# y9c/cutseq

Measured on AMD Instinct MI355X. Metric: M read-pairs/sec, higher is better.
Workload: dtype u8

## Files before the change

cutseq_amd/csrc/cutseq_hip.hip:

```cpp
#include <hip/hip_runtime.h>

#include <cstdarg>
#include <cstdio>
#include <cstdlib>
#include <cstring>
#include <algorithm>
#include <atomic>
#include <map>
#include <new>
#include <string>
#include <thread>
#include <vector>

#include <sys/mman.h>

#include "../../include/cutseq_hip.h"
#include "trim_kernel.hip.inc"
#include "long_kernel.hip.inc"
#include "text_kernels.hip.inc"
#include "deflate_kernels.hip.inc"
#include "info_kernels.hip.inc"

namespace {

// ... 82 lines not shown
}

struct cs_engine {
  int device = -1;
  hipStream_t stream = nullptr;
  int plan_slot = -1;
  hipStream_t resolve_stream = nullptr;
  unsigned long long *d_stats = nullptr;
  Lane lanes[kLanes];
  int next_lane = 0;
  Lane *last_lane = nullptr;
  uint32_t timed_calls = 0;
  double kernel_ms_total[2] = {0, 0};
  uint32_t max_reads = 0, max_stride = 0;
  bool paired = false;
  bool coded = false;
  bool wide = false;
  bool max_n = false;
  int n_cus = 256;
  uint32_t n_table_ops = 1;
  uint32_t col_dwords = 0;
  uint32_t waves_per_simd[2] = {4, 4};
  bool long_demux = false;
  int demux_mate = -1;
  uint32_t info_adapters = 0, info_max_m = 0, info_uniq_flags = 0;
  uint32_t demux_bins = 0;
  std::vector<Slot> slots;
  uint32_t max_dynamic_lds[2] = {0, 0};
  std::vector<void *> d_tables;
  uint32_t knob_col_bytes = 0, knob_grid_x = 0, knob_batch = 1;
  uint32_t knob_resolve_waves = 4;
  uint32_t knob_item_slots = 0;
  uint32_t knob_fast_recode = 1;
  bool knob_units = false;
  uint32_t knob_big_shift = 0, knob_small_shift = 0, knob_big_pct = 50;
};

namespace {

bool is_acgt(uint8_t c) { return c == 'A' || c == 'C' || c == 'G' || c == 'T'; }

void sync_fields(csdev::DevOp &d) {
  const cs_op &o = d.op;
  csdev::DevFields &f = d.f;
  f.kind = o.kind, f.align_flags = o.align_flags, f.reversed = o.reversed, f.remove = o.remove, f.shortcut = o.shortcut;
  f.match_flag = o.match_flag, f.required = o.required, f.conditional = o.conditional, f.capture = o.capture;
  f.homopolymer = o.homopolymer, f.q_base = o.q_base, f.stat_slot = o.stat_slot, f.m = o.m, f.k = o.k;
  f.min_overlap = o.min_overlap, f.force_min_len = o.force_min_len, f.cut_len = o.cut_len, f.q_cutoff = o.q_cutoff;
}

int build_dev_op(const cs_op &in, csdev::DevOp &out, int index, int mate) {
  memset(&out, 0, sizeof out);
  out.op = in;
  cs_op &op = out.op;
  switch (op.kind) {
    case CS_OP_ADAPTER: {
      if (op.m < 1 || op.m > CS_MAX_ADAPTER) return fail(CS_ERR_ARG, "mate %d op %d: adapter length %u", mate, index, op.m);
      if (op.min_overlap < 1 || op.min_overlap > op.m)
        return fail(CS_ERR_ARG, "mate %d op %d: min_overlap %u not in [1, m]", mate, index, op.min_overlap);
      if (op.align_flags > 15) return fail(CS_ERR_ARG, "mate %d op %d: bad align_flags", mate, index);
      if (op.k > op.m || op.thr[op.m] != op.k)
        return fail(CS_ERR_ARG, "mate %d op %d: k=%u inconsistent with thr[m]=%u", mate, index, op.k, op.thr[op.m]);
      for (int i = 1; i <= op.m; ++i)
        if (op.thr[i] < op.thr[i - 1] || op.thr[i] > op.thr[i - 1] + 1)
          return fail(CS_ERR_ARG, "mate %d op %d: thr[] must be a non-decreasing unit-step table", mate, index);
      if (op.remove > 1 || op.shortcut > 1) return fail(CS_ERR_ARG, "mate %d op %d: bad remove/shortcut", mate, index);
// ... 151 lines not shown
    a.mate[m].bc = rr[m]->bc;
    a.mate[m].xflags = rr[m]->xflags;
  }
  Lane &ln = eng->lanes[eng->next_lane];
  eng->next_lane = (eng->next_lane + 1) % kLanes;
  if (ln.used && hipEventQuery(ln.done) != hipSuccess) HIP_TRY(hipStreamWaitEvent(stream, ln.done, 0));
  if (n_reads > ln.defer_capacity) {
    const uint32_t cap = n_reads + n_reads / 8 + 1024;
    for (Lane &l : eng->lanes) {
      if (cap <= l.defer_capacity) continue;
      if (l.used) HIP_TRY(hipEventSynchronize(l.done));
      for (int m = 0; m < 2; ++m) {
        if (l.d_defer[m]) (void)hipFree(l.d_defer[m]);
        l.d_defer[m] = nullptr;
      }
      l.defer_capacity = 0;
      for (uint32_t m = 0; m < (eng->paired ? 2u : 1u); ++m)
        HIP_TRY(hipMalloc(&l.d_defer[m], (size_t)cap * kDeferRecordBytes));
      l.defer_capacity = cap;
    }
  }
  a.defer[0] = reinterpret_cast<uint4 *>(ln.d_defer[0]);
  a.defer[1] = reinterpret_cast<uint4 *>(ln.d_defer[1]);
  a.defer_count = ln.d_counters + kTileCounterDwords;
  a.defer_cap = ln.defer_capacity;
  a.stats = eng->d_stats;
  a.n_reads = n_reads;
  a.stride_dw = stride / 4;
  a.plan_slot = (uint32_t)eng->plan_slot;
  a.tile_counter = ln.d_counters;
  a.n_table_ops = eng->n_table_ops;
  a.batch_knob = eng->knob_batch;
  a.fast_recode = eng->knob_fast_recode;
  a.gate = gate;
  for (int mode = 0; mode < 2; ++mode)
    if (g[mode].lds_bytes > eng->max_dynamic_lds[mode]) {
      HIP_TRY(hipFuncSetAttribute(kernel_for(eng, mode), hipFuncAttributeMaxDynamicSharedMemorySize, (int)g[mode].lds_bytes));
      eng->max_dynamic_lds[mode] = g[mode].lds_bytes;
    }
  const uint32_t n_tiles = (n_reads + kTileRows - 1) / kTileRows;
  uint32_t gx[2];
  for (int mode = 0; mode < 2; ++mode) {
    uint32_t per_cu = kLdsBudget / g[mode].lds_bytes;
    const uint32_t wave_cap = 4 * eng->waves_per_simd[mode];
    if (per_cu > wave_cap) per_cu = wave_cap;
    if (per_cu < 1) per_cu = 1;
    if (mode == csdev::MODE_RESOLVE && rstream != stream && per_cu > eng->knob_resolve_waves) per_cu = eng->knob_resolve_waves;
    uint32_t resident = (uint32_t)eng->n_cus * per_cu * (mode == csdev::MODE_SCAN ? 2u : 1u);
    gx[mode] = resident / mates;
    if (mode == csdev::MODE_SCAN && eng->knob_grid_x) gx[mode] = eng->knob_grid_x;
    if (gx[mode] < 1) gx[mode] = 1;
    if (gx[mode] > n_tiles) gx[mode] = n_tiles;
  }
  a.static_units = gx[0] / 2 > 0 ? gx[0] / 2 : 1;
  const uint32_t share = n_tiles / a.static_units;
  a.big_shift = share >= 32 ? 3 : share >= 16 ? 2 : 1;
  a.small_shift = 0;
  uint32_t big_pct = 50;
  if (eng->knob_units) {
    a.big_shift = eng->knob_big_shift;
    a.small_shift = eng->knob_small_shift;
    big_pct = eng->knob_big_pct;
  }
  a.big_tiles = (uint32_t)((uint64_t)n_tiles * big_pct / 100) & ~((1u << a.big_shift) - 1u);
  if (time_it) {
    int rc = harvest(eng, ln);
// ... 572 lines not shown
  const size_t bytes = (size_t)max_reads * max_stride;
  for (Slot &s : eng->slots) {
    for (int m = 0; m < (eng->paired ? 2 : 1); ++m) {
      ENG_TRY(hipMalloc(&s.d_seq[m], bytes));
      ENG_TRY(hipMalloc(&s.d_qual[m], bytes));
      ENG_TRY(hipMalloc(&s.d_len[m], (size_t)max_reads * sizeof(uint16_t)));
      ENG_TRY(hipMalloc(&s.d_out[m], (size_t)max_reads * sizeof(cs_result)));
      ENG_TRY(hipMalloc(&s.d_bc[m], (size_t)max_reads));
      if (eng->max_n) ENG_TRY(hipMalloc(&s.d_xf[m], (size_t)max_reads));
    }
    ENG_TRY(hipMalloc(&s.d_cap2, (size_t)max_reads * sizeof(cs_cap2)));
    ENG_TRY(hipEventCreateWithFlags(&s.done, hipEventDisableTiming));
  }
  ENG_TRY(hipDeviceSynchronize());
#undef ENG_TRY
  for (int mode = 0; mode < 2; ++mode) {
    hipFuncAttributes fa;
    if (hipFuncGetAttributes(&fa, kernel_for(eng, mode)) == hipSuccess && fa.numRegs > 0) {
      const uint32_t alloc = ((uint32_t)fa.numRegs + 7u) / 8u * 8u;
      uint32_t w = 512u / alloc;
      eng->waves_per_simd[mode] = w < 1 ? 1 : (w > 8 ? 8 : w);
    }
  }
  if (const char *env = getenv("CUTSEQ_COL_BYTES")) {
    const long v = atol(env);
    if (v >= 1024 && v <= 32768) eng->knob_col_bytes = (uint32_t)v;
  }
  if (const char *env = getenv("CUTSEQ_BATCH_KNOB")) eng->knob_batch = (uint32_t)atol(env);
  if (const char *env = getenv("CUTSEQ_ITEM_SLOTS")) {
    const long v = atol(env);
    if (v >= 1 && v <= 16) eng->knob_item_slots = (uint32_t)v;
  }
  if (const char *env = getenv("CUTSEQ_FAST_RECODE")) eng->knob_fast_recode = (uint32_t)atoi(env) <= 2u ? (uint32_t)atoi(env) : 1u;
  if (const char *env = getenv("CUTSEQ_RESOLVE_WAVES")) {
    const long v = atol(env);
    if (v >= 1 && v <= 16) eng->knob_resolve_waves = (uint32_t)v;
  }
  if (const char *env = getenv("CUTSEQ_GRID_X")) {
    const long v = atol(env);
    if (v > 0) eng->knob_grid_x = (uint32_t)v;
  }
  if (const char *env = getenv("CUTSEQ_UNITS")) {
    unsigned bs, ss, pc;
    if (sscanf(env, "%u,%u,%u", &bs, &ss, &pc) == 3 && bs <= 6 && ss <= bs && pc <= 100) {
      eng->knob_units = true;
      eng->knob_big_shift = bs;
      eng->knob_small_shift = ss;
      eng->knob_big_pct = pc;
    }
  }
  *out = eng;
  return CS_OK;
}

int cs_trim_device(cs_engine *eng, void *stream, const cs_reads *r1, const cs_reads *r2, uint32_t n_reads,
                   uint32_t stride) {
  if (!eng || !r1) return fail(CS_ERR_ARG, "null engine or reads");
  HIP_TRY(hipSetDevice(eng->device));
  hipStream_t st = stream ? (hipStream_t)stream : eng->stream;
  return launch(eng, st, st, r1, r2, n_reads, stride, true);
}

int cs_trim_device_pipelined(cs_engine *eng, void *stream, const cs_reads *r1, const cs_reads *r2, uint32_t n_reads,
                             uint32_t stride) {
  if (!eng || !r1) return fail(CS_ERR_ARG, "null engine or reads");
  HIP_TRY(hipSetDevice(eng->device));
// ... 850 lines not shown
```

cutseq_amd/csrc/trim_kernel.hip.inc:

```

#include <type_traits>

namespace csdev {

#ifdef CS_PHASE_TIMERS
struct PhaseTimer {
  uint64_t last;
  uint32_t acc[8];
  uint32_t passes, steps, items;
};
#define CS_T_MARK(T, PHASE)                                   \
  {                                                           \
    const uint64_t cs_now = clock64();                        \
    (T).acc[PHASE] += (uint32_t)(cs_now - (T).last);          \
    (T).last = cs_now;                                        \
  }
#else
#define CS_T_MARK(T, PHASE)
#endif


constexpr int kWave = 64;

constexpr uint32_t kScoreBias = 1024u, kOriginBias = 4096u;
// ... 54 lines not shown

struct MateArgs {
  const uint32_t *seq;
  const uint8_t *qual;
  const uint16_t *len;
  cs_result *out;
  cs_cap2 *cap2;
  uint8_t *bc;
  uint8_t *xflags;
};

constexpr uint32_t kTileCounters = 8, kTileCounterStride = 32;

struct KArgs {
  MateArgs mate[2];
  unsigned long long *stats;
  uint32_t n_reads;
  uint32_t stride_dw;
  uint32_t lds_stride_dw;
  uint32_t col_dwords;
  uint32_t plan_slot;
  uint32_t *tile_counter;
  uint32_t n_table_ops;
  uint32_t big_tiles;
  uint32_t big_shift, small_shift;
  uint32_t static_units;
  uint4 *defer[2];
  uint32_t batch_knob;
  uint32_t *defer_count;
  uint32_t defer_cap;
  const unsigned long long *gate;
  uint32_t item_slots;
  uint32_t fast_recode;
};

__device__ __forceinline__ uint32_t cell_pack(int cost, int score, int origin) {
  return ((uint32_t)cost << kCostShift) | ((uint32_t)(score + (int)kScoreBias) << kScoreShift) |
         (uint32_t)(origin + (int)kOriginBias);
}
__device__ __forceinline__ int cell_cost(uint32_t c) { return (int)(c >> kCostShift); }
__device__ __forceinline__ int cell_score(uint32_t c) { return (int)((c >> kScoreShift) & 0x7ffu) - (int)kScoreBias; }
__device__ __forceinline__ int cell_origin(uint32_t c) { return (int)(c & 0x1fffu) - (int)kOriginBias; }
constexpr uint32_t kStripScoreBias = 256u, kStripPrioShift = 22;
constexpr uint32_t kStripZero = (kStripScoreBias << kScoreShift) | kOriginBias;
__device__ __forceinline__ uint32_t strip_pack(int cost, int score, int origin) {
  return ((uint32_t)cost << kCostShift) | ((uint32_t)(score + (int)kStripScoreBias) << kScoreShift) |
         (uint32_t)(origin + (int)kOriginBias);
}
__device__ __forceinline__ int strip_score(uint32_t c) {
  return (int)((c >> kScoreShift) & 0x1ffu) - (int)kStripScoreBias;
}

__device__ __forceinline__ int thr_of(const DevOp &d, int L) {
  if (d.thr_mul) return (int)(__umul24((uint32_t)max(L, 0), d.thr_mul) >> 16);
  if (L <= 0) return 0;
  if (L <= 64) return __popcll(d.thr_step[0] & (~0ull >> (64 - L)));
  return __popcll(d.thr_step[0]) + __popcll(d.thr_step[1] & (~0ull >> (128 - L)));
}
__device__ __forceinline__ int thr_step_bit(const DevOp &d, int i) {
  return (int)(((i <= 64) ? (d.thr_step[0] >> (i - 1)) : (d.thr_step[1] >> (i - 65))) & 1ull);
}

__device__ __forceinline__ uint32_t encode4_nib(uint32_t w) {
  const uint32_t sel = (w >> 1) & 0x03030303u;
  const uint32_t expect = __builtin_amdgcn_perm(0u, 0x47544341u , sel);
  const uint32_t diff = expect ^ w;
  const uint32_t nz = (((diff & 0x7f7f7f7fu) + 0x7f7f7f7fu) | diff) & 0x80808080u;
// ... 164 lines not shown
  const W Xh = (((Eq & Pv) + Pv) ^ Pv) | Eq;
  W Ph = Mv | ~(Xh | Pv);
  W Mh = Pv & Xh;
  st.score += (int)((Ph >> top_shift) & 1) - (int)((Mh >> top_shift) & 1);
  Ph = (Ph << 1) | hin;
  Mh = Mh << 1;
  st.Pv = Mh | ~(Xv | Ph);
  st.Mv = Ph & Xv;
}

__device__ __forceinline__ uint32_t shl1_full_rate(uint32_t x) {
  uint32_t r;
  asm("v_add_u32 %0, %1, %1" : "=v"(r) : "v"(x));
  return r;
}
constexpr uint32_t kTtA = 0xF0u, kTtB = 0xCCu, kTtC = 0xAAu;
template <bool HIN>
__device__ __forceinline__ void myers_step_la(MyersState<uint32_t> &st, uint32_t Eq, uint32_t hin_bit) {
  const uint32_t Pv = st.Pv, Mv = st.Mv;
  const uint32_t Xv = Eq | Mv;
  const uint32_t t = (Eq & Pv) + Pv;
  const uint32_t Xh = __builtin_amdgcn_bitop3_b32(t, Pv, Eq, ((kTtA ^ kTtB) | kTtC) & 0xFFu);
  const uint32_t Ph = __builtin_amdgcn_bitop3_b32(Mv, Xh, Pv, (kTtA | ~(kTtB | kTtC)) & 0xFFu);
  const uint32_t Mh = Pv & Xh;
  st.score += (int)(Ph >> 31) - (int)(Mh >> 31);
  uint32_t Ph2 = shl1_full_rate(Ph);
  if (HIN) Ph2 |= hin_bit;
  const uint32_t Mh2 = shl1_full_rate(Mh);
  st.Pv = __builtin_amdgcn_bitop3_b32(Mh2, Xv, Ph2, (kTtA | ~(kTtB | kTtC)) & 0xFFu);
  st.Mv = Ph2 & Xv;
}

typedef __attribute__((address_space(3))) const uint32_t lds_cu32;
__device__ __forceinline__ uint32_t lds_addr_of(const void *p) {
  return (uint32_t)(uintptr_t)(__attribute__((address_space(3))) const void *)p;
}
__device__ __forceinline__ uint32_t lds_read_u32(uint32_t addr) { return *(lds_cu32 *)(uintptr_t)addr; }

constexpr int kFnibDwords = 6;
#ifndef PRIO_LOOP
#define PRIO_LOOP 0
#define PRIO_REST 3
#define PRIO_RESOLVE 3
#endif
constexpr int kRingRecords = 16;

__device__ __forceinline__ int hamming_coded(const uint32_t *row, int p0, const uint32_t *fnib, int f0, int L, int m) {
  const int rw = p0 >> 3, fw = f0 >> 3;
  const uint32_t rsh = (uint32_t)(p0 & 7) * 4u, fsh = (uint32_t)(f0 & 7) * 4u;
  uint32_t rd[5], fd[5];
#pragma unroll
  for (int q = 0; q < 5; ++q) {
    if (8 * (q - 1) >= m) break;
    rd[q] = row[rw + q];
    fd[q] = fnib[fw + q];
  }
  int diff = 0;
#pragma unroll
  for (int q = 0; q < 4; ++q) {
    if (8 * q >= m) break;
    const uint32_t r = __builtin_amdgcn_alignbit(rd[q + 1], rd[q], rsh);
    const uint32_t f = __builtin_amdgcn_alignbit(fd[q + 1], fd[q], fsh);
    uint32_t x = r ^ f;
    x |= x >> 1;
    x |= x >> 2;
    x &= 0x11111111u;
// ... 560 lines not shown
    bool any = false;
    for (int i = skip + 1; i <= m; ++i) {
      cost += (int)(pv & 1u) - (int)(mv & 1u);
      pv >>= 1;
      mv >>= 1;
      thr_i += thr_step_bit(d, i);
      any = any || cost <= thr_i;
    }
    none = none && !any;
  }
  return none;
}

__device__ __forceinline__ unsigned long long lds_read_u64(uint32_t addr) { return *(const lds_u64 *)(uintptr_t)addr; }
typedef __attribute__((address_space(3))) uint8_t lds_u8;
__device__ __forceinline__ void lds_write_u8(uint32_t addr, uint32_t imm, uint32_t value) {
  *(lds_u8 *)(uintptr_t)(addr + imm) = (uint8_t)value;
}
__device__ __forceinline__ uint32_t lds_read_u8(uint32_t addr) { return *(const lds_u8 *)(uintptr_t)addr; }
__device__ __forceinline__ uint32_t pk_min_u16(uint32_t a, uint32_t b) {
  uint32_t r;
  asm("v_pk_min_u16 %0, %1, %2" : "=v"(r) : "v"(a), "v"(b));
  return r;
}

struct ItemLog {
  uint32_t slot0;
  uint32_t bytes;
  uint32_t tag_off;
};

template <bool HAS_A>
__device__ __forceinline__ Verdict myers_pair(const DevOp &da, const DevOp &db, int rule, const uint32_t *fnib_b,
                                               const uint32_t *row, int e, bool &a_none, const ItemLog &il CS_T_PARAM) {
  constexpr int NB = 8;
  constexpr int s = 0;
  const int n = e - s;
  const int m = db.f.m, k = db.f.k;
  const bool RS = db.f.align_flags & CS_REF_START;
  const int sh = 32 - m;
  MyersState<uint32_t> st;
  st.Mv = 0;
  st.Pv = RS ? 0u : (m >= 32 ? ~0u : ((1u << m) - 1u));
  const int k1 = k + 1;
  st.score = (RS ? 0 : m) - k1;
  st.Pv = (st.Pv << sh) | ((1u << sh) - 1u);
  const bool exact_by_score = !RS;
  int jfirst = -1, jlast = -1;
  int cmin = 0x7fff, jmin = -1;
  bool tie_next = false;
  uint32_t slot = il.slot0;
  const uint32_t slot_end = il.slot0 + il.bytes;
  bool log_full = false;
  const int ma = da.f.m, ka = da.f.k;
  const int sha = 32 - ma, free_a = ma - (int)da.f.min_overlap;
  MyersState<uint32_t> sa;
  sa.Mv = 0;
  sa.Pv = (((ma >= 32 ? ~0u : ((1u << ma) - 1u)) & ~((1u << free_a) - 1u)) << sha) | ((1u << sha) - 1u);
  sa.score = ma - free_a;
  int flag = 0;
  const uint32_t tn0 = da.pair_tn[0], tn1 = da.pair_tn[1], tn2 = da.pair_tn[2], tn3 = da.pair_tn[3];
  const uint32_t fill_a = (uint32_t)sha, cst4 = (uint32_t)(4 + 2 * ka + 1);
  auto sample_a = [&](uint32_t cst) {
    const int cur = (int)__builtin_popcount(sa.Pv) - (int)(__builtin_popcount(sa.Mv) + fill_a);
    flag |= sa.score + cur - (int)cst;
    sa.score = cur;
  };
  const unsigned long long tn_lo = ((unsigned long long)tn1 << 32) | tn0, tn_hi = ((unsigned long long)tn3 << 32) | tn2;
  auto tn_of = [tn_lo, tn_hi, ka](int j) -> int {
    int t1 = ka + 1;
    if (__ballot(j <= 32)) {
      const unsigned long long w = j <= 16 ? tn_lo : tn_hi;
      const int tj = (int)((uint32_t)(w >> (((uint32_t)(j - 1) & 15u) * 4u)) & 15u);
      t1 = j > 32 ? t1 : tj;
    }
    return t1;
  };
  auto column = [&](uint32_t eb, uint32_t ea, int j) {
    myers_step_la<false>(st, eb, 0u);
    if constexpr (HAS_A) {
      myers_step_la<false>(sa, ea, 0u);
      flag |= sa.score - tn_of(j);
    }
    if (st.score < 0) {
      if (jfirst < 0) jfirst = j;
      jlast = j;
      if (j == jmin + 1 && st.score + k1 == cmin) tie_next = true;
      if (st.score + k1 < cmin) {
        cmin = st.score + k1;
        jmin = j;
        tie_next = false;
      }
    }
  };
  int j = 1;
  if (n >= NB) {
    int wi = 0;
    auto take = [&]() -> uint32_t { return row[wi]; };
    auto advance = [&]() { wi += 1; };
#ifndef CS_PAIR_DEPTH
#define CS_PAIR_DEPTH 2
#endif
    constexpr int QD = CS_PAIR_DEPTH;
    static_assert(NB % QD == 0, "a group's columns must map onto the slots the same way in every group");
    uint32_t qb[QD], qa[QD];
    auto refill = [&](int slot, uint32_t code) {
      const unsigned long long pr = lds_read_u64(code);
      qb[slot] = (uint32_t)pr;
      qa[slot] = (uint32_t)(pr >> 32);
    };
    uint32_t wcur = take();
    advance();
#pragma unroll
    for (int u = 0; u < QD; ++u) refill(u, word_code<true>(wcur, u));
    auto group = [&](auto early_tag, uint32_t tw) {
      constexpr bool EARLY = decltype(early_tag)::value;
      const uint32_t wnext = take();
      advance();
      int sc[NB];
#pragma unroll
      for (int u = 0; u < NB; ++u) {
        myers_step_la<false>(st, qb[u % QD], 0u);
        sc[u] = st.score;
        if constexpr (HAS_A && EARLY) {
          myers_step_la<false>(sa, qa[u % QD], 0u);
          flag |= sa.score - (int)((tw >> (4 * u)) & 15u);
        } else if constexpr (HAS_A) {
          myers_step_noscore<false>(sa, qa[u % QD], 0u);
          if (u == 3 || u == 7) sample_a(cst4);
        }
        refill(u % QD, u + QD < NB ? word_code<true>(wcur, u + QD) : word_code<true>(wnext, u + QD - NB));
      }
      wcur = wnext;
      constexpr uint32_t kOr3 = 0xFEu;
      uint32_t any = __builtin_amdgcn_bitop3_b32((uint32_t)sc[0], (uint32_t)sc[1], (uint32_t)sc[2], kOr3);
      any = __builtin_amdgcn_bitop3_b32(any, (uint32_t)sc[3], (uint32_t)sc[4], kOr3);
      any = __builtin_amdgcn_bitop3_b32(any, (uint32_t)sc[5], (uint32_t)sc[6], kOr3);
      any |= (uint32_t)sc[7];
      if ((int)any < 0) {
        if (slot < slot_end) {
#pragma unroll
          for (int u = 0; u < NB; ++u) lds_write_u8(slot, (uint32_t)u, (uint32_t)sc[u]);
          lds_write_u8((slot >> 3) + il.tag_off, 0u, (uint32_t)(j >> 3));
        }
        slot += 8u;
      }
      j += NB;
    };
    __builtin_amdgcn_s_setprio(PRIO_LOOP);
    const int early_groups = (ma + ka + NB - 1) >> 3;
    if constexpr (HAS_A) {
      int g = 0;
      do {
        group(std::true_type{}, g == 0 ? tn0 : g == 1 ? tn1 : g == 2 ? tn2 : tn3);
        ++g;
      } while (g < early_groups && j + NB - 1 <= n);
    }
    while (j + NB - 1 <= n) group(std::false_type{}, 0u);
    __builtin_amdgcn_s_setprio(PRIO_REST);
    if (j <= n) {
      int sc[NB];
#pragma unroll
      for (int u = 0; u < NB - 1; ++u) {
        sc[u] = 0x7f;
        if (j + u <= n) {
          uint32_t eb, ea;
          if (u < QD) {
            eb = qb[u];
            ea = qa[u];
          } else {
            const unsigned long long pr = lds_read_u64(word_code<true>(wcur, u));
            eb = (uint32_t)pr;
            ea = (uint32_t)(pr >> 32);
          }
          myers_step_la<false>(st, eb, 0u);
          sc[u] = st.score;
          if constexpr (HAS_A) {
            myers_step_la<false>(sa, ea, 0u);
            flag |= sa.score - tn_of(j + u);
          }
        }
      }
      sc[NB - 1] = 0x7f;
      int any = sc[0];
#pragma unroll
      for (int u = 1; u < NB - 1; ++u) any |= sc[u];
      if (any < 0) {
        if (slot < slot_end) {
#pragma unroll
          for (int u = 0; u < NB; ++u) lds_write_u8(slot, (uint32_t)u, (uint32_t)sc[u]);
          lds_write_u8((slot >> 3) + il.tag_off, 0u, (uint32_t)(j >> 3));
        }
        slot += 8u;
      }
      j = n + 1;
    }
    {
      const uint32_t m80 = 0x80808080u, ones = 0x01010101u;
      const uint32_t stop_at = min(slot, slot_end);
      uint32_t rd = il.slot0;
      while (__ballot(rd < stop_at)) {
        if (rd < stop_at) {
          const unsigned long long sc8 = lds_read_u64(rd);
          const int jg = (int)lds_read_u8((rd >> 3) + il.tag_off) * 8 + 1;
          rd += 8u;
          const uint32_t clo = (uint32_t)sc8 & m80, chi = (uint32_t)(sc8 >> 32) & m80;
          const uint32_t plo = (uint32_t)sc8 ^ m80, phi = (uint32_t)(sc8 >> 32) ^ m80;
          const unsigned long long c64 = ((unsigned long long)chi << 32) | clo;
          if (jfirst < 0) jfirst = jg + (__builtin_ctzll(c64) >> 3);
          jlast = jg + ((63 - __builtin_clzll(c64)) >> 3);
          const uint32_t h00ff = 0x00ff00ffu;
          const uint32_t a0 = plo & h00ff, a1 = (plo >> 8) & h00ff, b0 = phi & h00ff, b1 = (phi >> 8) & h00ff;
          const uint32_t m4 = pk_min_u16(pk_min_u16(a0, a1), pk_min_u16(b0, b1));
          const uint32_t gbyte = min(m4 & 0xffffu, m4 >> 16);
          const int gmin = (int)gbyte - 128 + k1;
          if (jmin == jg - 1 && (int)(plo & 0xffu) - 128 + k1 == cmin) tie_next = true;
          if (gmin < cmin) {
            const uint32_t gb = __builtin_amdgcn_perm(0u, gbyte, 0u);
            const uint32_t xlo = plo ^ gb, xhi = phi ^ gb;
            const uint32_t zlo = (xlo - ones) & ~xlo & m80, zhi = (xhi - ones) & ~xhi & m80;
            const int pos = __builtin_ctzll(((unsigned long long)zhi << 32) | zlo) >> 3;
            cmin = gmin;
            jmin = jg + pos;
            const unsigned long long flipped = ((unsigned long long)phi << 32) | plo;
            tie_next = pos < 7 && (uint32_t)((flipped >> (8 * (pos + 1))) & 0xffull) == gbyte;
          }
        }
// ... 850 lines not shown
  const uint32_t big_mask = (1u << a.big_shift) - 1u, small_mask = (1u << a.small_shift) - 1u;
  auto unit_start = [&](uint32_t u) -> uint32_t {
    return (u < big_units) ? (u << a.big_shift) : big_tiles + ((u - big_units) << a.small_shift);
  };
  auto unit_end = [&](uint32_t tile) -> uint32_t {
    return (tile < big_tiles) ? ((tile | big_mask) + 1u) : big_tiles + (((tile - big_tiles) | small_mask) + 1u);
  };
  uint32_t *next_slot = sacc + kStatWords;
  const uint32_t n_counters = min(kTileCounters, (uint32_t)gridDim.x);
  const uint32_t my_counter = blockIdx.x % n_counters;
  uint32_t *counter = a.tile_counter + ((uint32_t)mate * kTileCounters + my_counter) * kTileCounterStride;
  uint32_t *claim = a.defer_count + (2u + (uint32_t)mate) * kTileCounterStride;
  auto next_unit = [&]() -> uint32_t { return a.static_units + my_counter + n_counters * atomicAdd(counter, 1u); };
  if (SCAN) {
    if (tid == 0) *next_slot = unit_start(blockIdx.x < a.static_units ? blockIdx.x : next_unit());
  } else {
    if (tid == 0) *next_slot = atomicAdd(claim, 1u);
  }
  __syncthreads();
  uint32_t tile_id = *next_slot, next_id = 0;
#ifdef CS_PHASE_TIMERS
  PhaseTimer pt;
  pt.last = clock64();
  for (int i = 0; i < 8; ++i) pt.acc[i] = 0;
  pt.passes = pt.steps = pt.items = 0;
#endif

  uint4 *ring = reinterpret_cast<uint4 *>((reinterpret_cast<uintptr_t>(sacc + kStatWords + 4) + 15u) & ~(uintptr_t)15u);
  uint32_t pend_count = 0;
  bool pend_asked = false;
  uint32_t pend_q = 0;
  auto flush_ring = [&]() {
    const uint32_t qb = (uint32_t)__builtin_amdgcn_readfirstlane((int)pend_q);
    if ((uint32_t)lane < pend_count) {
      uint4 *rec = a.defer[mate] + (size_t)(qb + (uint32_t)lane) * 2u;
      rec[0] = ring[lane * 2];
      rec[1] = ring[lane * 2 + 1];
    }
    pend_count = 0;
    pend_asked = false;
  };
  bool fast_ok = SCAN && CODED && a.fast_recode != 0u, fast_failed = false;
  for (; tile_id < n_tiles; tile_id = next_id) {
  uint32_t lane_fresh = threadIdx.x;
  asm volatile("" : "+v"(lane_fresh));
  const int tid = (int)lane_fresh, lane = tid;
  const bool top = !SCAN && tile_id >= tiles_a;
  const uint32_t row0 = top ? (tile_id - tiles_a) * (uint32_t)TILE : tile_id * batch_rows;
  const uint32_t rows_here = top ? min((uint32_t)TILE, n_refl - row0) : min(batch_rows, (SCAN ? a.n_reads : n_records) - row0);
  const bool valid = (uint32_t)tid < rows_here;

  uint32_t gr = row0 + tid;
  int s = 0, e = 0, t0 = 0;
  uint32_t fm = 0, capo = 0, qc = 0;
  uint32_t meta = (uint32_t)CS_DEMUX_NONE << 16;
  uint32_t rec_win = 0, rec_rows = 0, rec_rmax = 0;
  if (!SCAN) {
    uint4 ra = make_uint4(0, 0, 0, 0), rb = make_uint4(0, 0, 0, 0);
    if (valid) {
      const uint4 *rec = a.defer[mate] + (size_t)(top ? a.defer_cap - 1u - gr : gr) * 2u;
      ra = rec[0];
      rb = rec[1];
    }
    gr = ra.x;
    s = (int)(ra.y & 0xffffu);
    e = (int)(ra.y >> 16);
    rec_win = ra.z;
    rec_rows = ra.w;
    t0 = (int)(rb.x >> 24);
    fm = (rb.y & 0xffu) | ((rb.x & 0xffffffu) << 8);
    meta = ((rb.y >> 8) & 0xffu) | ((rb.w >> 24) << 16);
    rec_rmax = (rb.y >> 16) & 0xffu;
    capo = rb.z;
    qc = ((rb.w >> 8) & 0xffffu) | ((rb.y >> 24) << 16) | (rb.w << 24);
  }

  const uint32_t len_raw = valid ? (uint32_t)ma.len[gr] : 0u;
// ... 136 lines not shown
  if (tid == 0 && !same_unit) fetched = SCAN ? atomic_add_later(counter, 1u) : atomic_add_later(claim, 1u);
  if (SCAN && pend_count >= (uint32_t)kRingRecords / 2) {
    if (tid == 0) pend_q = atomic_add_later(&a.defer_count[mate * kTileCounterStride], pend_count);
    pend_asked = true;
  }
  const uint32_t *wave_rows = tile;
  const uint32_t *myrow = wave_rows + (size_t)lane * a.lds_stride_dw;
  bool deferred = false;
  bool refl = false;
  bool refl_any = false;
  uint32_t refl_q = 0, refl_rank = 0;

  if (SCAN) e = len;
  int t_first = 0;
  if constexpr (SCAN && CODED) {
    const bool pair = use_filter && n_ops >= 2 && plan->ops[mate][0].pair_next;
    const bool solo = use_filter && n_ops >= 1 && plan->ops[mate][0].solo_first;
    if (pair || solo) {
      const int tb = pair ? 1 : 0;
      const DevOp &da = plan->ops[mate][0], &db = plan->ops[mate][tb];
      if (lane < 8) {
        cur_tab[lane * 2] = tables[tb * (kEqTableBytes / 4) + lane * 2 + 1];
        cur_tab[lane * 2 + 1] = (pair && lane < 4) ? smem[16 + lane] : 0u;
      }
      wave_lds_fence();
      bool none = true;
      Verdict vb = verdict_none(db.f.m);
      if (here && len > 0) {
        ItemLog il;
        il.bytes = a.item_slots * 8u;
        il.slot0 = lds_addr_of(ring + kRingRecords * 2) + (uint32_t)lane * il.bytes;
        il.tag_off = (lds_addr_of(ring + kRingRecords * 2) + (uint32_t)TILE * il.bytes) - (lds_addr_of(ring + kRingRecords * 2) >> 3);
        if (pair)
          vb = myers_pair<true>(da, db, rule, fnibs + kFnibDwords, myrow, len, none, il CS_T_ARG);
        else
          vb = myers_pair<false>(da, db, rule, fnibs, myrow, len, none, il CS_T_ARG);
      }
      CS_T_MARK(pt, 2);
      refl = !none;
      const unsigned long long rm = __ballot(refl);
      if (rm) {
        if (lane == 0) refl_q = atomic_add_later(&a.defer_count[(4u + (uint32_t)mate) * kTileCounterStride], (uint32_t)__popcll(rm));
        refl_rank = __builtin_amdgcn_mbcnt_hi((uint32_t)(rm >> 32), __builtin_amdgcn_mbcnt_lo((uint32_t)rm, 0u));
        refl_any = true;
      }
      if (refl) {
        deferred = true;
        rec_win = 0;
        rec_rows = 0xffffffffu;
        rec_rmax = 0xffu;
      } else if (here) {
        if (pair && da.f.required) fm |= CS_F_UNTRIMMED;
#ifdef CS_EXP_REASON
        for (int q = 0; q < 24; ++q) {
          const unsigned long long bm = __ballot(vb.need && vb.reason == q);
          if (bm && lane == 0) atomicAdd(&a.stats[(size_t)mate * kStatWords + ST_OPS + 8 + (q % 12)], (unsigned long long)__popcll(bm) << (q >= 12 ? 32 : 0));
        }
#endif
        if (vb.need) {
          meta += 0x100u;
          deferred = true;
          meta = (meta & 0x00ffffffu) | ((uint32_t)tb << 24);
          rec_win = (uint32_t)vb.j0 | ((uint32_t)vb.j1 << 16) | ((uint32_t)vb.do_end << 31);
          rec_rows = vb.rows;
          rec_rmax = (uint32_t)vb.rmax;
        } else if (vb.found) {
          meta += 1u;
          fm |= (uint32_t)db.f.match_flag | (0x100u << tb);
          if (db.f.remove == CS_REMOVE_BEFORE)
// ... 486 lines not shown
    }
    if (ma.cap2) {
      cs_cap2 c2;
      c2.off = (uint16_t)(capo >> 16);
      c2.len = (uint8_t)(qc >> 24);
      c2._pad = 0;
      ma.cap2[gr] = c2;
    }
    if (ma.bc) ma.bc[gr] = (uint8_t)(meta >> 16);
  }

  if constexpr (MAXN) {
    bool many = false;
    if (fin) {
      uint32_t nn;
      if (SCAN && CODED && a.fast_recode == 1u && !fast_failed)
        nn = count_n_nibbles(myrow, s, e);
      else if (!CODED)
        nn = count_n_bytes(myrow, s, e);
      else
        nn = count_n_bytes(ma.seq + (size_t)gr * a.stride_dw, s, e);
      many = too_many_n(nn, e - s, plan->max_n);
    }
    const uint32_t w_many = wave_count(many);
    if (lane == 0 && w_many) atomicAdd(&sacc[ST_TOO_MANY_N], w_many);
    if (fin && ma.xflags) ma.xflags[gr] = many ? (uint8_t)CS_X_TOO_MANY_N : (uint8_t)0;
  }


  {
    const uint32_t w_reads = wave_count(fin);
    const bool narrow = a.stride_dw <= 255u;
    uint32_t w_in, w_out, w_qt, w_exact;
    if (narrow) {
      const uint32_t io = wave_sum(fin ? ((uint32_t)len | ((uint32_t)(e - s) << 16)) : 0u);
      const uint32_t qx = wave_sum((fin ? (qc & 0xffffu) : 0u) | (((meta >> 8) & 0xffu) << 16));
      w_in = io & 0xffffu, w_out = io >> 16, w_qt = qx & 0xffffu, w_exact = qx >> 16;
    } else {
      w_in = wave_sum(fin ? (uint32_t)len : 0u);
      w_out = wave_sum(fin ? (uint32_t)(e - s) : 0u);
      w_qt = wave_sum(fin ? (qc & 0xffffu) : 0u);
      w_exact = wave_sum((meta >> 8) & 0xffu);
    }
    const uint32_t w_short = wave_count(fin && (fm & CS_F_TOO_SHORT));
    const uint32_t w_untr = wave_count(fin && (fm & CS_F_UNTRIMMED));
    const uint32_t w_refilter = SCAN ? wave_count(deferred && rec_rmax == 0xffu) : 0u;
    if (lane == 0) {
      if (w_refilter) atomicAdd(&sacc[ST_RESERVED], w_refilter);
      atomicAdd(&sacc[ST_READS], w_reads);
      atomicAdd(&sacc[ST_IN_BP], w_in);
      atomicAdd(&sacc[ST_OUT_BP], w_out);
      atomicAdd(&sacc[ST_QTRIM_BP], w_qt);
      atomicAdd(&sacc[ST_TOO_SHORT], w_short);
      atomicAdd(&sacc[ST_UNTRIMMED], w_untr);
      atomicAdd(&sacc[ST_EXACT_DP], w_exact);
    }
    for (int t = 0; t < n_ops; ++t) {
      const unsigned long long bal = __ballot(fin && ((fm >> (8 + t)) & 1u));
      if (lane == 0 && bal) atomicAdd(&sacc[ST_OPS + plan->ops[mate][t].f.stat_slot], (uint32_t)__popcll(bal));
    }
  }

  if (SCAN && refl_any) {
    const uint32_t qb = (uint32_t)__builtin_amdgcn_readfirstlane((int)refl_q);
    if (refl) {
      uint4 ra, rb;
      ra.x = gr;
// ... 5 lines not shown
      rb.z = capo;
      rb.w = (qc >> 24) | ((qc & 0xffffu) << 8) | ((meta << 8) & 0xff000000u);
      uint4 *rec = a.defer[mate] + (size_t)(a.defer_cap - 1u - (qb + refl_rank)) * 2u;
      rec[0] = ra;
      rec[1] = rb;
    }
  }
  if (SCAN && pend_asked) flush_ring();
  if (SCAN && def_mask) {
    if (!park) q_pos = (uint32_t)__builtin_amdgcn_readfirstlane((int)q_pos);
    if (deferred && !refl) {
      const uint32_t rank = __builtin_amdgcn_mbcnt_hi((uint32_t)(def_mask >> 32),
                                                      __builtin_amdgcn_mbcnt_lo((uint32_t)def_mask, 0u));
      uint4 ra, rb;
      ra.x = gr;
      ra.y = (uint32_t)s | ((uint32_t)e << 16);
      ra.z = rec_win;
      ra.w = rec_rows;
      rb.x = (fm >> 8) | (meta & 0xff000000u);
      rb.y = (fm & 0xffu) | ((meta & 0xffu) << 8) | ((rec_rmax & 0xffu) << 16) | ((qc << 8) & 0xff000000u);
      rb.z = capo;
      rb.w = (qc >> 24) | ((qc & 0xffffu) << 8) | ((meta << 8) & 0xff000000u);
      uint4 *rec = park ? ring + (pend_count + rank) * 2u : a.defer[mate] + (size_t)(q_pos + rank) * 2u;
      rec[0] = ra;
      rec[1] = rb;
    }
    if (park) pend_count += (uint32_t)__popcll(def_mask);
  }
  next_id = same_unit ? tile_id + 1 : SCAN ? unit_start(a.static_units + my_counter + n_counters * fetched) : fetched;
  next_id = (uint32_t)__builtin_amdgcn_readfirstlane((int)next_id);
  __syncthreads();
  CS_T_MARK(pt, 6);
  }
  if (SCAN && pend_count) {
    if (!pend_asked && tid == 0) pend_q = atomicAdd(&a.defer_count[mate * kTileCounterStride], pend_count);
    flush_ring();
  }
#ifdef CS_PHASE_TIMERS
  if ((CS_PHASE_TIMERS == 1) == SCAN) {
    if (lane == 0)
      for (int i = 0; i < 8; ++i) atomicAdd(&sacc[ST_OPS + 16 + i], pt.acc[i] >> 6);
    if (lane == 0) {
      atomicAdd(&sacc[ST_OPS + 13], pt.passes);
      atomicAdd(&sacc[ST_OPS + 14], pt.steps);
      atomicAdd(&sacc[ST_OPS + 15], pt.items);
    }
  }
  __syncthreads();
#endif

  if (tid < kStatWords && sacc[tid])
    atomicAdd(&a.stats[(size_t)mate * kStatWords + tid], (unsigned long long)sacc[tid]);
}

}
```

Before: 4201.

## Add uniform-length wave fast paths for Myers loops, tail, and stats

When every lane in a wave has the same read length, the Myers column loops run a fixed group count instead of per-iteration bound checks. The tail step uses a specialized path, and the per-wave stats reduction derives input bp from the common length so one wave_sum is dropped. The ring flush now reads LDS with 128-bit vector loads, and the lane id is taken from mbcnt rather than threadIdx. The ballot checks add a small cost on tiles whose reads vary in length, and the new paths are enabled by default through an env knob.

```diff
diff --git a/cutseq_amd/csrc/cutseq_hip.hip b/cutseq_amd/csrc/cutseq_hip.hip
--- a/cutseq_amd/csrc/cutseq_hip.hip
+++ b/cutseq_amd/csrc/cutseq_hip.hip
@@ -138,6 +138,7 @@
   uint32_t knob_resolve_waves = 4;
   uint32_t knob_item_slots = 0;
   uint32_t knob_fast_recode = 1;
+  uint32_t knob_uniform_tiles = 7;
   bool knob_units = false;
   uint32_t knob_big_shift = 0, knob_small_shift = 0, knob_big_pct = 50;
 };
@@ -355,6 +356,7 @@
   a.n_table_ops = eng->n_table_ops;
   a.batch_knob = eng->knob_batch;
   a.fast_recode = eng->knob_fast_recode;
+  a.uniform_tiles = eng->knob_uniform_tiles;
   a.gate = gate;
   for (int mode = 0; mode < 2; ++mode)
     if (g[mode].lds_bytes > eng->max_dynamic_lds[mode]) {
@@ -993,6 +995,7 @@
     if (v >= 1 && v <= 16) eng->knob_item_slots = (uint32_t)v;
   }
   if (const char *env = getenv("CUTSEQ_FAST_RECODE")) eng->knob_fast_recode = (uint32_t)atoi(env) <= 2u ? (uint32_t)atoi(env) : 1u;
+  if (const char *env = getenv("CUTSEQ_UNIFORM_TILES")) eng->knob_uniform_tiles = (uint32_t)atoi(env) <= 7u ? (uint32_t)atoi(env) : 7u;
   if (const char *env = getenv("CUTSEQ_RESOLVE_WAVES")) {
     const long v = atol(env);
     if (v >= 1 && v <= 16) eng->knob_resolve_waves = (uint32_t)v;
diff --git a/cutseq_amd/csrc/trim_kernel.hip.inc b/cutseq_amd/csrc/trim_kernel.hip.inc
--- a/cutseq_amd/csrc/trim_kernel.hip.inc
+++ b/cutseq_amd/csrc/trim_kernel.hip.inc
@@ -110,7 +110,9 @@
   const unsigned long long *gate;
   uint32_t item_slots;
   uint32_t fast_recode;
+  uint32_t uniform_tiles;
 };
+enum { UT_LOOPS = 1u, UT_TAIL = 2u, UT_STATS = 4u };
 
 __device__ __forceinline__ uint32_t cell_pack(int cost, int score, int origin) {
   return ((uint32_t)cost << kCostShift) | ((uint32_t)(score + (int)kScoreBias) << kScoreShift) |
@@ -341,6 +343,12 @@
 }
 
 typedef __attribute__((address_space(3))) const uint32_t lds_cu32;
+typedef uint32_t u32x4 __attribute__((ext_vector_type(4)));
+typedef __attribute__((address_space(3))) const u32x4 lds_cu32x4;
+__device__ __forceinline__ uint4 lds_read_u128(uint32_t addr) {
+  const u32x4 v = *(lds_cu32x4 *)(uintptr_t)addr;
+  return make_uint4(v.x, v.y, v.z, v.w);
+}
 __device__ __forceinline__ uint32_t lds_addr_of(const void *p) {
   return (uint32_t)(uintptr_t)(__attribute__((address_space(3))) const void *)p;
 }
@@ -967,7 +975,7 @@
 
 template <bool HAS_A>
 __device__ __forceinline__ Verdict myers_pair(const DevOp &da, const DevOp &db, int rule, const uint32_t *fnib_b,
-                                               const uint32_t *row, int e, bool &a_none, const ItemLog &il CS_T_PARAM) {
+                                               const uint32_t *row, int e, bool &a_none, const ItemLog &il, uint32_t ut_parts CS_T_PARAM) {
   constexpr int NB = 8;
   constexpr int s = 0;
   const int n = e - s;
@@ -1011,6 +1019,10 @@
     }
     return t1;
   };
+  auto tn_uniform = [tn0, tn1, tn2, tn3, ka](int j) -> int {
+    const uint32_t w = j <= 8 ? tn0 : j <= 16 ? tn1 : j <= 24 ? tn2 : tn3;
+    return j > 32 ? ka + 1 : (int)((w >> (((uint32_t)(j - 1) & 7u) * 4u)) & 15u);
+  };
   auto column = [&](uint32_t eb, uint32_t ea, int j) {
     myers_step_la<false>(st, eb, 0u);
     if constexpr (HAS_A) {
@@ -1027,6 +1039,10 @@
         tie_next = false;
       }
     }
+  };
+  auto uniform_len = [&]() -> int {
+    const int n0 = __builtin_amdgcn_readfirstlane(n);
+    return (n0 >= NB && __ballot(n == n0) == ~0ull) ? n0 : 0;
   };
   int j = 1;
   if (n >= NB) {
@@ -1084,15 +1100,73 @@
     };
     __builtin_amdgcn_s_setprio(PRIO_LOOP);
     const int early_groups = (ma + ka + NB - 1) >> 3;
-    if constexpr (HAS_A) {
+    const int ul = (ut_parts & UT_LOOPS) ? uniform_len() : 0;
+    if (ul) {
+      const int groups = ul >> 3;
       int g = 0;
-      do {
-        group(std::true_type{}, g == 0 ? tn0 : g == 1 ? tn1 : g == 2 ? tn2 : tn3);
-        ++g;
-      } while (g < early_groups && j + NB - 1 <= n);
-    }
-    while (j + NB - 1 <= n) group(std::false_type{}, 0u);
+      if constexpr (HAS_A) {
+        const int early = min(early_groups, groups);
+        do {
+          group(std::true_type{}, g == 0 ? tn0 : g == 1 ? tn1 : g == 2 ? tn2 : tn3);
+          ++g;
+        } while (g < early);
+      }
+      for (; g < groups; ++g) group(std::false_type{}, 0u);
+    } else {
+      if constexpr (HAS_A) {
+        int g = 0;
+        do {
+          group(std::true_type{}, g == 0 ? tn0 : g == 1 ? tn1 : g == 2 ? tn2 : tn3);
+          ++g;
+        } while (g < early_groups && j + NB - 1 <= n);
+      }
+      while (j + NB - 1 <= n) group(std::false_type{}, 0u);
+    }
     __builtin_amdgcn_s_setprio(PRIO_REST);
+    auto log_tail = [&](const int (&sc)[NB], int any, uint32_t tag) {
+      if (any < 0) {
+        if (slot < slot_end) {
+#pragma unroll
+          for (int u = 0; u < NB; ++u) lds_write_u8(slot, (uint32_t)u, (uint32_t)sc[u]);
+          lds_write_u8((slot >> 3) + il.tag_off, 0u, tag);
+        }
+        slot += 8u;
+      }
+    };
+    const int ut = (ut_parts & UT_TAIL) ? uniform_len() : 0;
+    if (ut) {
+      const int tl = ut & (NB - 1), ju = (ut & ~(NB - 1)) + 1;
+      if (tl) {
+        int sc[NB];
+#pragma unroll
+        for (int u = 0; u < NB - 1; ++u) {
+          sc[u] = 0x7f;
+          if (u < tl) {
+            uint32_t eb, ea;
+            if (u < QD) {
+              eb = qb[u];
+              ea = qa[u];
+            } else {
+              const unsigned long long pr = lds_read_u64(word_code<true>(wcur, u));
+              eb = (uint32_t)pr;
+              ea = (uint32_t)(pr >> 32);
+            }
+            myers_step_la<false>(st, eb, 0u);
+            sc[u] = st.score;
+            if constexpr (HAS_A) {
+              myers_step_la<false>(sa, ea, 0u);
+              flag |= sa.score - tn_uniform(ju + u);
+            }
+          }
+        }
+        sc[NB - 1] = 0x7f;
+        int any = sc[0];
+#pragma unroll
+        for (int u = 1; u < NB - 1; ++u) any |= sc[u];
+        log_tail(sc, any, (uint32_t)(ju >> 3));
+      }
+      j = n + 1;
+    }
     if (j <= n) {
       int sc[NB];
 #pragma unroll
@@ -1120,14 +1194,7 @@
       int any = sc[0];
 #pragma unroll
       for (int u = 1; u < NB - 1; ++u) any |= sc[u];
-      if (any < 0) {
-        if (slot < slot_end) {
-#pragma unroll
-          for (int u = 0; u < NB; ++u) lds_write_u8(slot, (uint32_t)u, (uint32_t)sc[u]);
-          lds_write_u8((slot >> 3) + il.tag_off, 0u, (uint32_t)(j >> 3));
-        }
-        slot += 8u;
-      }
+      log_tail(sc, any, (uint32_t)(j >> 3));
       j = n + 1;
     }
     {
@@ -2044,17 +2111,20 @@
   uint32_t pend_q = 0;
   auto flush_ring = [&]() {
     const uint32_t qb = (uint32_t)__builtin_amdgcn_readfirstlane((int)pend_q);
-    if ((uint32_t)lane < pend_count) {
-      uint4 *rec = a.defer[mate] + (size_t)(qb + (uint32_t)lane) * 2u;
-      rec[0] = ring[lane * 2];
-      rec[1] = ring[lane * 2 + 1];
+    uint32_t ln = __builtin_amdgcn_mbcnt_hi(~0u, __builtin_amdgcn_mbcnt_lo(~0u, 0u));
+    asm volatile("" : "+v"(ln));
+    if (ln < pend_count) {
+      uint4 *rec = a.defer[mate] + (size_t)(qb + ln) * 2u;
+      const uint32_t src = lds_addr_of(ring) + ln * 32u;
+      rec[0] = lds_read_u128(src);
+      rec[1] = lds_read_u128(src + 16u);
     }
     pend_count = 0;
     pend_asked = false;
   };
   bool fast_ok = SCAN && CODED && a.fast_recode != 0u, fast_failed = false;
   for (; tile_id < n_tiles; tile_id = next_id) {
-  uint32_t lane_fresh = threadIdx.x;
+  uint32_t lane_fresh = __builtin_amdgcn_mbcnt_hi(~0u, __builtin_amdgcn_mbcnt_lo(~0u, 0u));
   asm volatile("" : "+v"(lane_fresh));
   const int tid = (int)lane_fresh, lane = tid;
   const bool top = !SCAN && tile_id >= tiles_a;
@@ -2257,9 +2327,9 @@
         il.slot0 = lds_addr_of(ring + kRingRecords * 2) + (uint32_t)lane * il.bytes;
         il.tag_off = (lds_addr_of(ring + kRingRecords * 2) + (uint32_t)TILE * il.bytes) - (lds_addr_of(ring + kRingRecords * 2) >> 3);
         if (pair)
-          vb = myers_pair<true>(da, db, rule, fnibs + kFnibDwords, myrow, len, none, il CS_T_ARG);
+          vb = myers_pair<true>(da, db, rule, fnibs + kFnibDwords, myrow, len, none, il, a.uniform_tiles CS_T_ARG);
         else
-          vb = myers_pair<false>(da, db, rule, fnibs, myrow, len, none, il CS_T_ARG);
+          vb = myers_pair<false>(da, db, rule, fnibs, myrow, len, none, il, a.uniform_tiles CS_T_ARG);
       }
       CS_T_MARK(pt, 2);
       refl = !none;
@@ -2812,7 +2882,17 @@
     const uint32_t w_reads = wave_count(fin);
     const bool narrow = a.stride_dw <= 255u;
     uint32_t w_in, w_out, w_qt, w_exact;
-    if (narrow) {
+    bool eq_tile = false;
+    int len0 = 0;
+    if (SCAN && narrow && (a.uniform_tiles & UT_STATS)) {
+      len0 = __builtin_amdgcn_readfirstlane(len);
+      eq_tile = len0 >= 8 && __ballot(here && len == len0) == ~0ull;
+    }
+    if (eq_tile) {
+      const uint32_t oq = wave_sum(fin ? ((uint32_t)(e - s) | ((qc & 0xffffu) << 16)) : 0u);
+      w_in = w_reads * (uint32_t)len0, w_out = oq & 0xffffu, w_qt = oq >> 16;
+      w_exact = wave_count((meta & 0xff00u) != 0u);
+    } else if (narrow) {
       const uint32_t io = wave_sum(fin ? ((uint32_t)len | ((uint32_t)(e - s) << 16)) : 0u);
       const uint32_t qx = wave_sum((fin ? (qc & 0xffffu) : 0u) | (((meta >> 8) & 0xffu) << 16));
       w_in = io & 0xffffu, w_out = io >> 16, w_qt = qx & 0xffffu, w_exact = qx >> 16;
@@ -2884,8 +2964,11 @@
   __syncthreads();
   CS_T_MARK(pt, 6);
   }
+  uint32_t tid_end_u = __builtin_amdgcn_mbcnt_hi(~0u, __builtin_amdgcn_mbcnt_lo(~0u, 0u));
+  asm volatile("" : "+v"(tid_end_u));
+  const int tid_end = (int)tid_end_u;
   if (SCAN && pend_count) {
-    if (!pend_asked && tid == 0) pend_q = atomicAdd(&a.defer_count[mate * kTileCounterStride], pend_count);
+    if (!pend_asked && tid_end == 0) pend_q = atomicAdd(&a.defer_count[mate * kTileCounterStride], pend_count);
     flush_ring();
   }
 #ifdef CS_PHASE_TIMERS
@@ -2901,8 +2984,8 @@
   __syncthreads();
 #endif
 
-  if (tid < kStatWords && sacc[tid])
-    atomicAdd(&a.stats[(size_t)mate * kStatWords + tid], (unsigned long long)sacc[tid]);
-}
-
-}
+  if (tid_end < kStatWords && sacc[tid_end])
+    atomicAdd(&a.stats[(size_t)mate * kStatWords + tid_end], (unsigned long long)sacc[tid_end]);
+}
+
+}
```

Result: no change. 4196 (-0.1%).
